# bio-phys/BioEn

Measured on NVIDIA B200. Metric: grad_evals_per_s, higher is better.
Workload: dtype f64

## Files before the change

bioen_b200/csrc/bioen_b200.cu:

```cuda
#include "../../include/bioen_b200.h"

#include <chrono>
#include <cmath>
#include <limits>
#include <memory>
#include <mutex>

#include "batched.cuh"
#include "context.cuh"
#include "gsl_min.cuh"
#include "lbfgs.cuh"

using namespace bioen;

namespace {
thread_local std::string g_last_error;
thread_local int g_error_pending = 0;
int g_fast_flag = 0;

void set_error(const char* where, const std::exception& e) {
    g_last_error = std::string(where) + ": " + e.what();
    g_error_pending = 1;
    fprintf(stderr, "%s\n", g_last_error.c_str());
}
// ... 262 lines not shown
            case BIOEN_B200_OPT_LAZY_GRADIENT: ctx->C.lazy_gradient = value != 0; break;
            case BIOEN_B200_OPT_P2P:
                if (ctx->comm) {
                    if (ctx->comm->is_local() && !value)
                        throw std::invalid_argument("bioen_b200: an in-process group has no NCCL path");
                    ctx->comm->use_p2p = value != 0;
                }
                break;
            case BIOEN_B200_OPT_FUSED_EXCHANGE: ctx->C.fuse_allowed = value != 0; break;
            case BIOEN_B200_OPT_PERSISTENT: ctx->C.persistent_mode = value; break;
            case BIOEN_B200_OPT_LBFGS_GRAM: ctx->C.lbfgs_gram_opt = value != 0; break;
            case BIOEN_B200_OPT_SLICE: ctx->C.slice_mode = value; break;
            case BIOEN_B200_OPT_LBFGS_SMALL: ctx->C.lbfgs_small_opt = value != 0; break;
            case BIOEN_B200_OPT_LBFGS_SPECULATIVE: ctx->C.lbfgs_speculative = value != 0; break;
            case BIOEN_B200_OPT_FETCH_ZEROCOPY: ctx->C.fetch_zero_copy = value != 0; break;
            case BIOEN_B200_OPT_STRUCTURE_MAJOR_ONLY:
                CUDA_CHECK(cudaSetDevice(ctx->C.device));
                if (value) ctx->C.enter_yt_only();
                else if (ctx->C.yt_only)
                    throw std::invalid_argument("bioen_b200: the row-major matrix is gone; create a new context");
                break;
            case BIOEN_B200_OPT_FP32_STORAGE:
                CUDA_CHECK(cudaSetDevice(ctx->C.device));
                ctx->pending_gen = -1;
                if (value) ctx->C.convert_to_fp32();
                else if (ctx->C.storage_fp32)
                    throw std::invalid_argument("bioen_b200: the fp64 matrix was released; upload yTilde again");
                break;
            default: throw std::invalid_argument("bioen_b200: unknown option");
        }
// ... 883 lines not shown
```

bioen_b200/csrc/common.cuh:

```cuda
#pragma once
#include <cuda.h>
#include <cuda_runtime.h>
#include <nvtx3/nvToolsExt.h>
#include <stdint.h>

#include <cstdio>
#include <stdexcept>
#include <string>

namespace bioen {

struct CudaError : std::runtime_error {
    using std::runtime_error::runtime_error;
};

inline void cuda_check(cudaError_t e, const char* what, const char* file, int line) {
    if (e != cudaSuccess) {
        char buf[512];
        snprintf(buf, sizeof buf, "bioen_b200: CUDA error %d (%s) at %s:%d: %s", (int)e, cudaGetErrorString(e),
                 file, line, what);
        throw CudaError(buf);
    }
}
#define CUDA_CHECK(x) ::bioen::cuda_check((x), #x, __FILE__, __LINE__)
// ... 78 lines not shown
}

__device__ __forceinline__ void bulk_load_1d_hint(void* dst, const void* src, uint32_t bytes, uint64_t* bar,
                                                  uint64_t policy) {
    asm volatile(
        "cp.async.bulk.shared::cluster.global.mbarrier::complete_tx::bytes.L2::cache_hint [%0], [%1], %2, [%3], %4;" ::
            "r"(smem_u32(dst)),
        "l"(reinterpret_cast<uint64_t>(src)), "r"(bytes), "r"(smem_u32(bar)), "l"(policy)
        : "memory");
}

__device__ __forceinline__ void prefetch_tensormap(const CUtensorMap* map) {
    asm volatile("prefetch.tensormap [%0];" ::"l"(reinterpret_cast<uint64_t>(map)) : "memory");
}

__device__ __forceinline__ double warp_sum(double v) {
#pragma unroll
    for (int o = 16; o > 0; o >>= 1) v += __shfl_xor_sync(0xffffffffu, v, o);
    return v;
}

__device__ __forceinline__ double warp_max(double v) {
#pragma unroll
    for (int o = 16; o > 0; o >>= 1) v = fmax(v, __shfl_xor_sync(0xffffffffu, v, o));
    return v;
}

template <int K>
__device__ __forceinline__ void block_sum(double (&v)[K], double* red) {
    const int lane = threadIdx.x & 31, wid = threadIdx.x >> 5, nw = (blockDim.x + 31) >> 5;
// ... 114 lines not shown
```

bioen_b200/csrc/context.cuh:

```cuda
#pragma once
#include <cstdlib>
#include <cstring>
#include <string>
#include <thread>
#include <vector>

#include "comm.cuh"
#include "fused_pass.cuh"
#include <atomic>
#include "persistent_eval.cuh"
#include "slice_eval.cuh"
#include "stream_pass.cuh"
#include "vector_kernels.cuh"

namespace bioen {

template <class T>
struct DevBuf {
    T* p = nullptr;
    size_t n = 0;
    DevBuf() = default;
    DevBuf(const DevBuf&) = delete;
    DevBuf& operator=(const DevBuf&) = delete;
    ~DevBuf() { release(); }
// ... 88 lines not shown

    DevBuf<double> Yt, fpart, flse;
    DevBuf<double> lbfgs_store;
    DevBuf<double> lbfgs_gram, lbfgs_gram_partials;
    bool lbfgs_gram_opt = false;
    bool lbfgs_small_opt = true;
    bool lbfgs_speculative = true;
    long long ldt = 0, f_nslab = 0, f_chunk = 0;
    int f_C = 0, f_stages = 0, f_grid = 0, f_KI = 0, f_smem = 0, f_T = 1, f_rows = 0, f_rows_per_cta = 1;
    bool f_team = false;
    bool fused_ready = false, yt_valid = false;
    bool allow_fused = true;
    double theta = 0.0;
    bool have_logw = false, have_forces = false;
    long long passes_launched = 0, kernels_launched = 0;

    Context(int m, int n, int dev, cudaStream_t user_stream = nullptr) : M(m), N(n), N_total(n), device(dev) {
        if (m <= 0 || n <= 0) throw std::invalid_argument("bioen_b200: matrix dimensions must be positive");
        CUDA_CHECK(cudaSetDevice(device));
        cudaDeviceProp prop;
        CUDA_CHECK(cudaGetDeviceProperties(&prop, device));
        if (prop.major < 10)
            throw CudaError("bioen_b200: this library is built for sm_100a (Blackwell B200) only");
        num_sms = prop.multiProcessorCount;
        if (user_stream) {
            stream = user_stream;
            own_stream = false;
        } else {
            CUDA_CHECK(cudaStreamCreateWithFlags(&stream, cudaStreamNonBlocking));
        }
// ... 47 lines not shown
                                        cudaFuncAttributeMaxDynamicSharedMemorySize, kPassSmemBytes));
        CUDA_CHECK(cudaFuncSetAttribute(stream_pass_kernel<kRowPass, false, float>,
                                        cudaFuncAttributeMaxDynamicSharedMemorySize, kPassSmemBytesF32));
        CUDA_CHECK(cudaFuncSetAttribute(stream_pass_kernel<kRowPass, true, float>,
                                        cudaFuncAttributeMaxDynamicSharedMemorySize, kPassSmemBytesF32));
        CUDA_CHECK(cudaFuncSetAttribute(stream_pass_kernel<kColPass, false, float>,
                                        cudaFuncAttributeMaxDynamicSharedMemorySize, kPassSmemBytesF32));
        CUDA_CHECK(cudaFuncSetAttribute(stream_pass_kernel<kColPass, true, float>,
                                        cudaFuncAttributeMaxDynamicSharedMemorySize, kPassSmemBytesF32));
        CUDA_CHECK(cudaFuncSetAttribute(stream_colgrad_kernel<double>, cudaFuncAttributeMaxDynamicSharedMemorySize,
                                        kPassSmemBytes));
        CUDA_CHECK(cudaFuncSetAttribute(stream_colgrad_kernel<float>, cudaFuncAttributeMaxDynamicSharedMemorySize,
                                        kPassSmemBytesF32));
        colgrad_part.alloc((size_t)grid * 3 + 8);
        if (const char* e = getenv("BIOEN_B200_COLGRAD")) colgrad_opt = e[0] != '0';
        CUDA_CHECK(cudaFuncSetAttribute(persistent_eval_kernel<double>, cudaFuncAttributeMaxDynamicSharedMemorySize,
                                        kPassSmemBytes));
        CUDA_CHECK(cudaFuncSetAttribute(persistent_eval_kernel<float>, cudaFuncAttributeMaxDynamicSharedMemorySize,
                                        kPassSmemBytesF32));
        pe_part.alloc((size_t)grid * kPSlots + 16);
        pe_bar.alloc(32);
        {
            int coop = 0, per_sm = 0;
            CUDA_CHECK(cudaDeviceGetAttribute(&coop, cudaDevAttrCooperativeLaunch, device));
            CUDA_CHECK(cudaOccupancyMaxActiveBlocksPerMultiprocessor(&per_sm, persistent_eval_kernel<float>,
                                                                     kPEvalThreads, kPassSmemBytesF32));
            coop_ok = coop && (long long)per_sm * num_sms >= grid;
            if (const char* e = getenv("BIOEN_B200_PERSISTENT")) persistent_mode = atoi(e);
            if (const char* e = getenv("BIOEN_B200_LBFGS_GRAM")) lbfgs_gram_opt = e[0] == '1';
            if (const char* e = getenv("BIOEN_B200_FETCH")) fetch_zero_copy = strcmp(e, "memcpy") != 0;
// ... 43 lines not shown
        lbfgs_gram_opt = getenv("BIOEN_B200_LBFGS_GRAM") != nullptr && getenv("BIOEN_B200_LBFGS_GRAM")[0] == '1';
        lbfgs_small_opt = !(getenv("BIOEN_B200_LBFGS_SMALL") && getenv("BIOEN_B200_LBFGS_SMALL")[0] == '0');
        persistent_mode = -1;
        if (const char* e = getenv("BIOEN_B200_PERSISTENT")) persistent_mode = atoi(e);
        slice_mode = -1;
        if (const char* e = getenv("BIOEN_B200_SLICE")) slice_mode = atoi(e);
        comm = nullptr;
        nranks = 1;
        N_total = N;
        Y = nullptr;
        storage_fp32 = false;
        Y32.release();
        yt_only = false;
        passes_launched = kernels_launched = 0;
        pass_timing = false;
    }
    void set_comm(Comm* c) {
        comm = c;
        nranks = c ? c->nranks : 1;
        if (nranks > 64) throw std::invalid_argument("bioen_b200: at most 64 ranks");
    }

    void upload_matrix(const double* host, size_t ld_host) {
        NvtxRange nvtx("bioen:upload_ytilde");
        ld = round_up(N, 16);
        if (Yown.n != (size_t)M * ld || !Yown.p) {
            Yown.release();
            CUDA_CHECK(cudaMalloc(&Yown.p, (size_t)M * ld * sizeof(double)));
            Yown.n = (size_t)M * ld;
        }
// ... 472 lines not shown
        P2PDev d{};
        d.nranks = 1;
        return d;
    }

    const double* lse_pairs() const { return nranks > 1 ? lse_all.p : sc.p + SC_LSE_MAX; }

    void launch_lse(double* x, const double* xp, const double* d, double stp, const double* w0, bool from_col,
                    const double* stp_dev = nullptr) {
        LseArgs a{};
        a.n = N; a.x = x; a.xp = xp; a.d = d; a.stp = stp; a.stp_dev = stp_dev; a.w0 = w0;
        a.col_partial = from_col ? partialB.p : nullptr;
        a.col_ld = Npad; a.col_L = nRT; a.col_chunk = col_chunk();
        a.write_xnorm = from_col ? 0 : 1;
        a.partials = red_partials.p; a.ticket = ticket.p; a.sc = sc.p;
        k_update_lse<<<vec_blocks_n, kVecThreads, 0, stream>>>(a);
        ++kernels_launched;
    }
    void gather_lse() {
        if (nranks > 1) comm->allgather(sc.p + SC_LSE_MAX, lse_all.p, 2, stream);
    }
    template <int MODE, bool SUB>
    void launch_pass(const double* vN, const double* vMb) {
        PassArgs a{};
        a.nRT = nRT; a.nCB = nCB; a.T = T; a.chunk = chunk;
        a.interleave = ((MODE == kRowPass) ? interleave_row : interleave_col) ? 1 : 0;
        a.evict_first = evict_first;
        a.vN = vN; a.vMb = vMb; a.ab = ab.p;
        a.partial = (MODE == kRowPass) ? partialA.p : partialB.p;
        a.ld = (MODE == kRowPass) ? Mpad : Npad;
        require_row_major("this evaluation path (tile kernels)");
        if (!has_matrix()) throw std::logic_error("bioen_b200: yTilde has not been uploaded");
        const bool timed = pass_timing && pass_ev_used + 2 <= pass_ev.size();
        if (timed) CUDA_CHECK(cudaEventRecord(pass_ev[pass_ev_used++], stream));
        if (storage_fp32)
            stream_pass_kernel<MODE, SUB, float><<<grid, kPassThreads, kPassSmemBytesF32, stream>>>(tmap, a);
        else
            stream_pass_kernel<MODE, SUB, double><<<grid, kPassThreads, kPassSmemBytes, stream>>>(tmap, a);
        if (timed) CUDA_CHECK(cudaEventRecord(pass_ev[pass_ev_used++], stream));
        CUDA_CHECK(cudaGetLastError());
        ++passes_launched;
        ++kernels_launched;
    }
    std::vector<cudaEvent_t> pass_ev;
    size_t pass_ev_used = 0;
    long long pass_ev_passes = 0;
    bool pass_timing = false;
    void begin_pass_timing(int max_passes) {
        while (pass_ev.size() < (size_t)max_passes * 2) {
            cudaEvent_t e;
            CUDA_CHECK(cudaEventCreate(&e));
            pass_ev.push_back(e);
        }
        pass_ev_used = 0;
        pass_ev_passes = 0;
        pass_timing = true;
    }
    float end_pass_timing() {
        pass_timing = false;
        sync();
        double total = 0.0;
        size_t cnt = 0;
        for (size_t i = 0; i + 1 < pass_ev_used; i += 2) {
            float t = 0.f;
            CUDA_CHECK(cudaEventElapsedTime(&t, pass_ev[i], pass_ev[i + 1]));
            total += t;
            ++cnt;
        }
        return cnt ? (float)(total / (double)(cnt + pass_ev_passes)) : 0.f;
    }
    void finalize_rows(bool is_forces, int ntail, bool ab_with_avg) {
        FinalizeArgs a{};
        a.m = M; a.partial = partialA.p; a.ld = Mpad; a.L = nCB; a.chunk = row_chunk();
        a.Y = Yobs.p; a.ab = ab.p; a.avg = avg.p; a.ab_with_avg = ab_with_avg ? 1 : 0;
        a.is_forces = is_forces ? 1 : 0; a.theta = theta;
        a.partials = red_partials.p; a.ticket = ticket.p; a.sc = sc.p;
        a.tail = msum.p + M;
        if (nranks > 1) {
            k_reduce_row_slots<<<vec_blocks_m, kVecThreads, 0, stream>>>(M, partialA.p, Mpad, nCB, row_chunk(), msum.p);
            ++kernels_launched;
            comm->allreduce_sum(msum.p, M + ntail, stream);
            a.msum = msum.p;
        }
        k_finalize_rows<<<(M + kVecThreads - 1) / kVecThreads, kVecThreads, 0, stream>>>(a);
        ++kernels_launched;
    }

    bool slice_ok() const {
        return slice_pl.ok && slice_coop && slice_mode != 0 && persistent_mode != 0 && nranks == 1 && Y != nullptr &&
               !storage_fp32 && (ld % 2) == 0 && ld >= N && (reinterpret_cast<uintptr_t>(Y) & 15) == 0;
    }
    void launch_slice(int method, int mode, double* x, const double* xp, const double* d, double stp,
                      const double* stp_dev, double* grad, const double* ddir) {
        SliceArgs a{};
        a.method = method; a.mode = mode; a.M = M; a.N = N;
        a.nc = slice_pl.nc; a.ncs = slice_pl.ncs; a.ms = slice_pl.ms;
        a.cx_log2 = slice_pl.cx_log2; a.l_log2 = slice_pl.l_log2; a.lt_log2 = slice_pl.lt_log2;
        a.Y = Y; a.ld = ld;
        a.x = x; a.xp = xp; a.d = d; a.stp = stp; a.stp_dev = stp_dev;
// ... 114 lines not shown
        ++eval_gen;
        if (persistent_for(false)) {
            launch_persistent(0, kPEvalObjective, x, xp, d, stp, stp_dev, nullptr, nullptr);
            eval_fused = nranks > 1;
            return;
        }
        launch_lse(x, xp, d, stp, nullptr, false, stp_dev);
        const bool fused = fuse_exchange();
        eval_fused = fused;
        if (!fused) gather_lse();
        {
            LogwWeightsArgs a{};
            a.n = N; a.g = x; a.G = Gv.p; a.w = w.p; a.lse_pairs = lse_pairs(); a.nranks = nranks;
            a.msum_tail = msum.p + M; a.partials = red_partials.p; a.ticket = ticket.p; a.sc = sc.p;
            a.local_only = fused ? 1 : 0;
            k_logw_weights<<<vec_blocks_n, kVecThreads, 0, stream>>>(a);
            ++kernels_launched;
        }
        launch_pass<kRowPass, false>(w.p, nullptr);
        if (fused) {
            RowsExchangeArgs a{};
            a.m = M; a.partial = partialA.p; a.ld = Mpad; a.L = nCB; a.chunk = row_chunk(); a.msum = msum.p;
            a.p2p = p2p_dev(); a.Y = Yobs.p; a.ab = ab.p; a.avg = avg.p; a.theta = theta; a.sc = sc.p;
            k_logw_rows_exchange_finalize<<<1, kRowsXThreads, 0, stream>>>(a);
            ++kernels_launched;
        } else {
            finalize_rows(false, 3, true);
        }
    }
    bool colgrad_eligible() const {
        return colgrad_opt && (nranks == 1 || fuse_exchange()) && interleave_col && !persistent_for(false);
// ... 1 lines not shown
    bool eval_fused = false;
    void logw_eval_g(const double* x, double* grad, const double* ddir) {
        NvtxRange nvtx("bioen:logw_eval_g");
        if (persistent_for(false) && (nranks == 1 || eval_fused)) {
            launch_persistent(0, kPEvalGradient, const_cast<double*>(x), nullptr, nullptr, 0.0, nullptr, grad, ddir);
            eval_fused = false;
            return;
        }
        auto aligned16 = [](const void* q) { return (reinterpret_cast<uintptr_t>(q) & 15) == 0; };
        const bool sharded_fused = nranks > 1 && eval_fused;
        if (colgrad_opt && (nranks == 1 || sharded_fused) && interleave_col && aligned16(x) && aligned16(grad) &&
            aligned16(Gv.p) && aligned16(w.p)) {
            PassArgs pa{};
            pa.nRT = nRT; pa.nCB = nCB; pa.T = T; pa.chunk = chunk; pa.interleave = 1; pa.evict_first = evict_first;
            pa.ab = ab.p; pa.partial = partialB.p; pa.ld = Npad;
            ColGradArgs ga{};
            ga.n = N; ga.g = x; ga.G = Gv.p; ga.w = w.p; ga.d = ddir; ga.grad = grad; ga.theta = theta; ga.sc = sc.p;
            ga.i_gbar = SC_GBAR; ga.i_Gbar = SC_CAPGBAR; ga.cta_part = colgrad_part.p;
            ga.i_wscale = sharded_fused ? SC_WSCALE : -1;
            ga.wio = w.p;
            const bool timed = pass_timing && pass_ev_used + 2 <= pass_ev.size();
            if (timed) CUDA_CHECK(cudaEventRecord(pass_ev[pass_ev_used++], stream));
            if (storage_fp32)
                stream_colgrad_kernel<float><<<grid, kPassThreads, kPassSmemBytesF32, stream>>>(tmap, pa, ga);
            else
                stream_colgrad_kernel<double><<<grid, kPassThreads, kPassSmemBytes, stream>>>(tmap, pa, ga);
            if (timed) CUDA_CHECK(cudaEventRecord(pass_ev[pass_ev_used++], stream));
            CUDA_CHECK(cudaGetLastError());
            if (sharded_fused) k_colgrad_finish_sharded<<<1, 256, 0, stream>>>(grid, colgrad_part.p, sc.p, p2p_dev());
            else k_colgrad_finish<<<1, 256, 0, stream>>>(grid, colgrad_part.p, sc.p, SC_DG, SC_GNORM2, SC_GINF);
            ++passes_launched;
            kernels_launched += 2;
            eval_fused = false;
            return;
        }
        launch_pass<kColPass, true>(nullptr, nullptr);
        {
            LogwGradArgs a{};
            a.n = N; a.col_partial = partialB.p; a.ld = Npad; a.L = nRT; a.chunk = col_chunk();
            a.g = x; a.G = Gv.p; a.w = w.p; a.d = ddir; a.grad = grad; a.theta = theta;
            a.partials = red_partials.p; a.ticket = ticket.p; a.sc = sc.p;
            a.wio = w.p;
            if (eval_fused) a.p2p = p2p_dev(); else a.p2p.nranks = 1;
            k_logw_grad<<<vec_blocks_n, kVecThreads, 0, stream>>>(a);
            ++kernels_launched;
// ... 212 lines not shown
```

bioen_b200/csrc/lbfgs.cuh:

```cuda
#pragma once
#include <chrono>
#include <cmath>
#include <cstdio>
#include <map>

#include "context.cuh"

namespace bioen {

enum {
    LBFGS_SUCCESS = 0,
    LBFGS_STOP = 1,
    LBFGS_ALREADY_MINIMIZED = 2,
    LBFGSERR_UNKNOWNERROR = -1024,
    LBFGSERR_LOGICERROR,
    LBFGSERR_OUTOFMEMORY,
    LBFGSERR_CANCELED,
    LBFGSERR_INVALID_N,
    LBFGSERR_INVALID_N_SSE,
    LBFGSERR_INVALID_X_SSE,
    LBFGSERR_INVALID_EPSILON,
    LBFGSERR_INVALID_TESTPERIOD,
    LBFGSERR_INVALID_DELTA,
    LBFGSERR_INVALID_LINESEARCH,
// ... 429 lines not shown
    LineSearchState* spec_ls = nullptr;
    bool take_spec_slope() {
        if (!spec_slope) return false;
        spec_slope = false;
        const double dg0 = C.h_sc[SC_DGINIT];
        spec_ls->set_slope(dg0);
        spec_bad = 0 < dg0;
        return spec_bad;
    }

    void enqueue_update(int end_old, int bound, int m) {
        NvtxRange nvtx("bioen:lbfgs_update(pair+two_loop)");
        const bool fused = reduce && C.fuse_exchange();
        PairArgs a{n, x, g, xp, gp, S[end_old], Yv[end_old], end_old, C.red_partials.p, C.ticket.p, C.sc.p, {}};
        if (fused) a.p2p = C.p2p_dev(); else a.p2p.nranks = 1;
        k_lbfgs_pair<<<vec_blocks, kVecThreads, 0, C.stream>>>(a);
        ++C.kernels_launched;
        if (reduce && !fused) {
            C.comm->allreduce_sum(C.sc.p + SC_YS, 2, C.stream);
            C.d2d(C.sc.p + SC_YS0 + end_old, C.sc.p + SC_YS, 1);
        }
        two_loop(bound, (end_old + 1) % m, m);
    }
    void enqueue_update_gram(int end_old, int bound) {
        NvtxRange nvtx("bioen:lbfgs_update(gram)");
        GramPairArgs a{};
        a.n = n; a.x = x; a.g = g; a.xp = xp; a.gp = gp;
        for (int t = 0; t < kGramM; ++t) { a.S[t] = S[t]; a.Y[t] = Yv[t]; }
        a.end = end_old; a.bound = bound; a.gram = C.lbfgs_gram.p; a.partials = C.lbfgs_gram_partials.p;
        a.ticket = C.ticket.p; a.sc = C.sc.p;
        if (reduce && C.fuse_exchange()) a.p2p = C.p2p_dev(); else a.p2p.nranks = 1;
// ... 41 lines not shown
                }
                it = g_update.emplace(key, std::make_pair(ex, nk)).first;
            }
            CUDA_CHECK(cudaGraphLaunch(it->second.first, C.stream));
            C.kernels_launched += it->second.second;
            return;
        }
        enqueue_update(end_old, bound, m);
    }

    void two_loop(int bound, int end, int m) {
        const bool fused = reduce && C.fuse_exchange();
        auto launch = [&](TwoLoopArgs& a) {
            a.n = n; a.d = d; a.g = g; a.partials = C.red_partials.p; a.ticket = C.ticket.p; a.sc = C.sc.p;
            if (fused && a.v) a.p2p = C.p2p_dev(); else a.p2p.nranks = 1;
            k_lbfgs_twoloop<<<vec_blocks, kVecThreads, 0, C.stream>>>(a);
            ++C.kernels_launched;
            if (reduce && !fused && a.v) C.comm->allreduce_sum(C.sc.p + a.out, 1, C.stream);
        };
        std::vector<int> js(bound);
        int j = end;
        for (int i = 0; i < bound; ++i) { j = (j + m - 1) % m; js[i] = j; }
        {
            TwoLoopArgs a{};
            a.init = 1; a.u = nullptr; a.c_num = a.c_den = 0; a.c2_num = -1; a.s_num = -1;
            a.v = S[js[0]]; a.out = SC_ALPHA0 + js[0];
            launch(a);
        }
        for (int i = 0; i < bound; ++i) {
            TwoLoopArgs a{};
            a.u = Yv[js[i]]; a.c_num = SC_ALPHA0 + js[i]; a.c_den = SC_YS0 + js[i]; a.csign = -1.0; a.c2_num = -1;
// ... 53 lines not shown
```

bioen_b200/csrc/stream_pass.cuh:

```cuda
#pragma once
#include "common.cuh"

namespace bioen {

enum PassMode { kRowPass = 0, kColPass = 1 };

constexpr int kTileR = 32;
constexpr int kTileC = 128;
#ifndef BIOEN_PASS_STAGES
#define BIOEN_PASS_STAGES 4
#endif
#ifndef BIOEN_PASS_CTAS_PER_SM
#define BIOEN_PASS_CTAS_PER_SM 1
#endif
constexpr int kStages = BIOEN_PASS_STAGES;
constexpr int kPassCtasPerSM = BIOEN_PASS_CTAS_PER_SM;
constexpr int kConsumerWarps = 8;
constexpr int kAuxBytes = 2048;
constexpr int kTileBytes = kTileR * kTileC * (int)sizeof(double);
constexpr int kStageBytes = kTileBytes + kAuxBytes;
constexpr int kPassThreads = (kConsumerWarps + 1) * 32;

template <typename T>
struct PassGeom {
// ... 5 lines not shown
constexpr int kPassSmemBytes = PassGeom<double>::kSmem;
constexpr int kPassSmemBytesF32 = PassGeom<float>::kSmem;

struct PassArgs {
    int nRT;
    int nCB;
    long long T;
    long long chunk;
    int interleave;
    int evict_first;
    const double* vN;
    const double* vMb;
    const double* ab;
    double* partial;
    long long ld;
};

__host__ __device__ inline long long pass_first_cta(long long run, long long L, long long chunk) {
    return chunk < 0 ? 0 : (run * L) / chunk;
}
__host__ __device__ inline int pass_num_slots(long long run, long long L, long long chunk) {
    if (chunk < 0) return (int)(-chunk);
    return (int)(((run + 1) * L - 1) / chunk - (run * L) / chunk) + 1;
}

struct TileWalk {
    long long run, left, L;
    int k, G, mode;
    __host__ __device__ __forceinline__ void init(int pass_mode, const PassArgs& a, int b, int grid) {
        L = (pass_mode == kRowPass) ? a.nCB : a.nRT;
// ... 75 lines not shown
        if (MODE == kRowPass) bytes += kTileC * 8 + (SUB ? kTileR * 8 : 0);
        else bytes += kTileR * 16;
        mbar_expect_tx(&full[stage], bytes);
        tma_load_2d(st, tmap, cb * kTileC, rt * kTileR, &full[stage], policy);
        if (MODE == kRowPass) {
            bulk_load_1d(st + kTileBytes, a.vN + (size_t)cb * kTileC, kTileC * 8, &full[stage]);
            if (SUB)
                bulk_load_1d(st + kTileBytes + kTileC * 8, a.vMb + (size_t)rt * kTileR, kTileR * 8, &full[stage]);
        } else {
            bulk_load_1d(st + kTileBytes, a.ab + (size_t)rt * kTileR * 2, kTileR * 16, &full[stage]);
        }
        if (++stage == kStages) { stage = 0; phase ^= 1; }
    }
    rp.stage = stage;
    rp.phase = phase;
}

template <typename T>
struct RowFrag;
template <>
struct RowFrag<double> {
    double2 v0, v1;
    __device__ __forceinline__ void load_v(const double2* vv, int lane) { v0 = vv[lane]; v1 = vv[32 + lane]; }
    __device__ __forceinline__ double dot(const unsigned char* rowp, int lane, bool sub, double b, double s) const {
        const double2* yr = reinterpret_cast<const double2*>(rowp);
        double2 y0 = yr[lane], y1 = yr[32 + lane];
        if (sub) { y0.x -= b; y0.y -= b; y1.x -= b; y1.y -= b; }
        s = fma(y0.x, v0.x, s);
        s = fma(y0.y, v0.y, s);
        s = fma(y1.x, v1.x, s);
// ... 121 lines not shown
    double* wio;
};

template <typename T>
__global__ void __launch_bounds__(kPassThreads, kPassCtasPerSM)
    stream_colgrad_kernel(const __grid_constant__ CUtensorMap tmap, const PassArgs a, const ColGradArgs ga) {
    using Geo = PassGeom<T>;
    constexpr int kNS = Geo::kNStages, kStageB = Geo::kStage, kTileB = Geo::kTile;
    constexpr int kRowBytes = kTileC * (int)sizeof(T);
    extern __shared__ __align__(1024) unsigned char smem_raw[];
    unsigned char* smem = smem_raw + ((128u - (smem_u32(smem_raw) & 127u)) & 127u);
    __shared__ double s_red[3][kConsumerWarps];
    const int warp = threadIdx.x >> 5, lane = threadIdx.x & 31;
    TileWalk tw;
    tw.init(kColPass, a, (int)blockIdx.x, (int)gridDim.x);
    pass_ring_init<T>(smem);
    __syncthreads();
    if (warp == kConsumerWarps) {
        if (lane == 0 && tw.left > 0) {
            prefetch_tensormap(&tmap);
            RingPos rp{0, 1};
            pass_produce<kColPass, true, T>(smem, &tmap, a, tw, rp);
        }
        return;
    }
    uint64_t* full = reinterpret_cast<uint64_t*>(smem + kNS * kStageB);
    uint64_t* empty = full + kNS;
    constexpr int CPW = kTileC / kConsumerWarps;
    const int cp = lane & 7, rg = lane >> 3;
    const double gbar = ga.sc[ga.i_gbar], Gbar = ga.sc[ga.i_Gbar];
    const double wscale = ga.i_wscale >= 0 ? ga.sc[ga.i_wscale] : 1.0;
// ... 62 lines not shown
            acc0 = acc1 = 0.0;
        }
    }
    dg = warp_sum(dg);
    gn = warp_sum(gn);
    gi = warp_max(gi);
    if (lane == 0) { s_red[0][warp] = dg; s_red[1][warp] = gn; s_red[2][warp] = gi; }
    asm volatile("bar.sync 1, %0;" ::"n"(kConsumerWarps * 32) : "memory");
    if (threadIdx.x == 0) {
        double t0 = 0.0, t1 = 0.0, t2 = 0.0;
        for (int w = 0; w < kConsumerWarps; ++w) { t0 += s_red[0][w]; t1 += s_red[1][w]; t2 = fmax(t2, s_red[2][w]); }
        ga.cta_part[3 * blockIdx.x + 0] = t0;
        ga.cta_part[3 * blockIdx.x + 1] = t1;
        ga.cta_part[3 * blockIdx.x + 2] = t2;
    }
}

__global__ void __launch_bounds__(256) k_colgrad_finish(int ncta, const double* cta_part, double* sc, int i_dg,
                                                        int i_gn, int i_gi) {
    __shared__ double red[3][8];
    double t0 = 0.0, t1 = 0.0, t2 = 0.0;
    for (int b = threadIdx.x; b < ncta; b += 256) {
        t0 += cta_part[3 * b];
        t1 += cta_part[3 * b + 1];
        t2 = fmax(t2, cta_part[3 * b + 2]);
    }
    t0 = warp_sum(t0); t1 = warp_sum(t1); t2 = warp_max(t2);
    if ((threadIdx.x & 31) == 0) { red[0][threadIdx.x >> 5] = t0; red[1][threadIdx.x >> 5] = t1; red[2][threadIdx.x >> 5] = t2; }
    __syncthreads();
    if (threadIdx.x == 0) {
        for (int w = 1; w < 8; ++w) { t0 += red[0][w]; t1 += red[1][w]; t2 = fmax(t2, red[2][w]); }
        sc[i_dg] = t0;
        sc[i_gn] = t1;
        sc[i_gi] = t2;
    }
}

template <int MODE, bool SUB, typename T = double>
__global__ void __launch_bounds__(kPassThreads, kPassCtasPerSM)
    stream_pass_kernel(const __grid_constant__ CUtensorMap tmap, const PassArgs a) {
    extern __shared__ __align__(1024) unsigned char smem_raw[];
    unsigned char* smem = smem_raw + ((128u - (smem_u32(smem_raw) & 127u)) & 127u);
    const int warp = threadIdx.x >> 5, lane = threadIdx.x & 31;
    TileWalk tw;
    tw.init(MODE, a, (int)blockIdx.x, (int)gridDim.x);
    pass_ring_init<T>(smem);
    __syncthreads();
    if (warp == kConsumerWarps) {
        if (lane == 0 && tw.left > 0) {
            prefetch_tensormap(&tmap);
            RingPos rp{0, 1};
            pass_produce<MODE, SUB, T>(smem, &tmap, a, tw, rp);
        }
        return;
    }
    if (tw.left == 0) return;
    RingPos rp{0, 0};
    pass_consume<MODE, SUB, T>(smem, a, tw, rp);
}

}
```

bioen_b200/csrc/vector_kernels.cuh:

```cuda
#pragma once
#include <float.h>

#include "comm.cuh"
#include "common.cuh"
#include "stream_pass.cuh"

namespace bioen {

enum ScalarSlot {
    SC_LSE_MAX = 0,
    SC_LSE_SUM = 1,
    SC_KL = 2,
    SC_GMAX = 3,
    SC_S = 4,
    SC_LOGS0 = 5,
    SC_GBAR = 6,
    SC_CAPGBAR = 7,
    SC_F = 8,
    SC_CHI2 = 9,
    SC_PRIOR = 10,
    SC_DG = 11,
    SC_GNORM2 = 12,
    SC_XNORM2 = 13,
    SC_WSCALE = 14,
// ... 63 lines not shown
    double stp;
    const double* stp_dev;
    const double* w0;
    const double* col_partial;
    long long col_ld;
    long long col_L, col_chunk;
    int write_xnorm;
    double* partials;
    unsigned int* ticket;
    double* sc;
};

__global__ void __launch_bounds__(kVecThreads) k_update_lse(const LseArgs a) {
    __shared__ double red[3 * 32];
    __shared__ bool is_last;
    double m = -DBL_MAX, s = 0.0, xn = 0.0;
    const double stp = a.stp_dev ? __ldg(a.stp_dev) : a.stp;
    for (int j = blockIdx.x * blockDim.x + threadIdx.x; j < a.n; j += gridDim.x * blockDim.x) {
        double x;
        if (a.col_partial) {
            const long long cb = j / kTileC;
            const int ns = pass_num_slots(cb, a.col_L, a.col_chunk);
            x = 0.0;
            for (int q = 0; q < ns; ++q) x += a.col_partial[(size_t)q * a.col_ld + j];
            a.x[j] = x;
        } else if (a.xp) {
            x = fma(stp, a.d[j], a.xp[j]);
            a.x[j] = x;
        } else {
            x = a.x[j];
// ... 43 lines not shown
    int n;
    const double* g;
    const double* G;
    double* w;
    const double* lse_pairs;
    int nranks;
    double* msum_tail;
    double* partials;
    unsigned int* ticket;
    double* sc;
    int local_only;
};

__global__ void __launch_bounds__(kVecThreads) k_logw_weights(const LogwWeightsArgs a) {
    __shared__ double red[3 * 32];
    double M, S;
    if (a.local_only) { M = a.sc[SC_LSE_MAX]; S = 1.0; }
    else global_lse(a.lse_pairs, a.nranks, M, S);
    const double inv = 1.0 / S;
    double v[3] = {0.0, 0.0, 0.0};
    for (int j = blockIdx.x * blockDim.x + threadIdx.x; j < a.n; j += gridDim.x * blockDim.x) {
        const double g = a.g[j], G = a.G[j];
        const double w = exp(g - M) * inv;
        a.w[j] = w;
        v[0] = fma(g - G, w, v[0]);
        v[1] = fma(g, w, v[1]);
        v[2] = fma(G, w, v[2]);
    }
    double* tail = a.msum_tail;
    double* sc = a.sc;
// ... 102 lines not shown
    const double* msum;
    const double* tail;
    const double* Y;
    double* ab;
    double* avg;
    int ab_with_avg;
    int is_forces;
    double theta;
    double* partials;
    unsigned int* ticket;
    double* sc;
};

__global__ void __launch_bounds__(kVecThreads) k_finalize_rows(const FinalizeArgs a) {
    __shared__ double red[32];
    double v[1] = {0.0};
    const int i = blockIdx.x * blockDim.x + threadIdx.x;
    if (i < a.m) {
        double s;
        if (a.msum) {
            s = a.msum[i];
        } else {
            const int ns = pass_num_slots(i / kTileR, a.L, a.chunk);
            s = 0.0;
            for (int q = 0; q < ns; ++q) s += a.partial[(size_t)q * a.ld + i];
        }
        const double r = s - a.Y[i];
        a.avg[i] = s;
        reinterpret_cast<double2*>(a.ab)[i] = make_double2(r, a.ab_with_avg ? s : 0.0);
        v[0] = r * r;
// ... 288 lines not shown
    }
    int fail;
    const double* in = p2p_deliver_and_wait(p, xs, K, &fail);
    if (threadIdx.x == 0) {
#pragma unroll
        for (int k = 0; k < K; ++k) {
            double s = 0.0;
            for (int r = 0; r < p.nranks; ++r) s += __ldcg(in + r * p.cap + k);
            v[k] = fail ? p2p_nan() : s;
        }
    }
}

__global__ void __launch_bounds__(kVecThreads) k_lbfgs_pair(const PairArgs a) {
    __shared__ double red[2 * 32];
    double v[2] = {0.0, 0.0};
    for (int j = blockIdx.x * blockDim.x + threadIdx.x; j < a.n; j += gridDim.x * blockDim.x) {
        const double x = a.x[j], g = a.g[j];
        const double s = x - a.xp[j], y = g - a.gp[j];
        a.s[j] = s;
        a.y[j] = y;
        a.xp[j] = x;
        a.gp[j] = g;
        v[0] = fma(y, s, v[0]);
        v[1] = fma(y, y, v[1]);
    }
    if (!grid_sum_last<2>(v, a.partials, a.ticket, red)) return;
    if (a.p2p.nranks > 1) p2p_sum_inline<2>(a.p2p, v);
    if (threadIdx.x == 0) {
        a.sc[SC_YS] = v[0];
// ... 9 lines not shown
    int init;
    const double* u;
    int c_num, c_den; double csign;
    int c2_num, c2_den; double c2sign;
    int s_num, s_den;
    const double* v;
    int out;
    double* partials;
    unsigned int* ticket;
    double* sc;
    P2PDev p2p;
};

__global__ void __launch_bounds__(kVecThreads) k_lbfgs_twoloop(const TwoLoopArgs a) {
    __shared__ double red[32];
    double coef = 0.0, scale = 1.0;
    if (a.u) {
        coef = a.csign * (a.sc[a.c_num] / a.sc[a.c_den]);
        if (a.c2_num >= 0) coef += a.c2sign * (a.sc[a.c2_num] / a.sc[a.c2_den]);
    }
    if (a.s_num >= 0) scale = a.sc[a.s_num] / a.sc[a.s_den];
    double v[1] = {0.0};
    for (int j = blockIdx.x * blockDim.x + threadIdx.x; j < a.n; j += gridDim.x * blockDim.x) {
        double dj = a.init ? -a.g[j] : a.d[j];
        if (a.u) dj = fma(coef, a.u[j], dj);
        if (a.s_num >= 0) dj *= scale;
        a.d[j] = dj;
        if (a.v) v[0] = fma(a.v[j], dj, v[0]);
    }
    if (a.v) {
// ... 482 lines not shown
```

include/bioen_b200.h:

```cpp
#ifndef BIOEN_B200_H
#define BIOEN_B200_H

#include <stddef.h>

#ifdef __cplusplus
extern "C" {
#endif


typedef struct params_t {
    double *forces;
    double *w0;
    double *g;
    double *G;
    double *yTilde;
    double *YTilde;
    double *w;
    double *result;
    double theta;
    double *yTildeT;
    int caching;
    double *tmp_n;
    double *tmp_m;
    int m;
// ... 77 lines not shown
int bioen_b200_adopt_ytilde(bioen_b200_ctx *ctx, double *yTilde_dev, size_t ld);
int bioen_b200_upload_rows(bioen_b200_ctx *ctx, int row0, int nrows, const double *rows_host, size_t ld);
void *bioen_b200_host_alloc(size_t bytes);
void bioen_b200_host_free(void *p);
int bioen_b200_alloc_ytilde(bioen_b200_ctx *ctx);
int bioen_b200_download_ytilde(bioen_b200_ctx *ctx, int row0, int nrows, long long col0, long long ncols,
                               double *out_host);

int bioen_b200_set_logw(bioen_b200_ctx *ctx, const double *G_host, const double *YTilde_host, double theta);
int bioen_b200_set_forces(bioen_b200_ctx *ctx, const double *w0_host, const double *YTilde_host, double theta);
int bioen_b200_set_theta(bioen_b200_ctx *ctx, double theta);
enum { BIOEN_B200_OPT_FUSED_FORCES = 1, BIOEN_B200_OPT_P2P = 2, BIOEN_B200_OPT_LAZY_GRADIENT = 3,
       BIOEN_B200_OPT_FUSED_EXCHANGE = 4, BIOEN_B200_OPT_PERSISTENT = 5, BIOEN_B200_OPT_LBFGS_GRAM = 6,
       BIOEN_B200_OPT_FP32_STORAGE = 7, BIOEN_B200_OPT_SLICE = 8, BIOEN_B200_OPT_LBFGS_SMALL = 9,
       BIOEN_B200_OPT_LBFGS_SPECULATIVE = 10, BIOEN_B200_OPT_STRUCTURE_MAJOR_ONLY = 11,
       BIOEN_B200_OPT_FETCH_ZEROCOPY = 12 };
int bioen_b200_set_option(bioen_b200_ctx *ctx, int option, int value);

int bioen_b200_eval(bioen_b200_ctx *ctx, int method, const double *x_host, double *f, double *grad_host);
int bioen_b200_grad_continue(bioen_b200_ctx *ctx, int method, double *grad_host);
int bioen_b200_weights(bioen_b200_ctx *ctx, int method, const double *x_host, double *w_host, double *sum);
int bioen_b200_average(bioen_b200_ctx *ctx, const double *w_host, double *avg_host);
int bioen_b200_affine_rows(bioen_b200_ctx *ctx, const double *scale_host, const double *offset_host);
int bioen_b200_forces_from_weights(bioen_b200_ctx *ctx, const double *w_host, double *f, double *grad_host);

int bioen_b200_opt_lbfgs(bioen_b200_ctx *ctx, int method, const double *x0_host, double *x_host,
                         lbfgs_config_params config, visual_params visual, double *fmin, int info[4]);
int bioen_b200_opt_gsl(bioen_b200_ctx *ctx, int method, const double *x0_host, double *x_host,
                       gsl_config_params config, visual_params visual, double *fmin, int info[4]);

int bioen_b200_theta_scan(bioen_b200_ctx *ctx, int method, int K, const double *thetas, const double *x0_host,
// ... 45 lines not shown
```

Baseline: 438.7.

## Use programmatic dependent launch to overlap kernel prologues with predecessors

Launches the pass, colgrad, vector and L-BFGS kernels through cudaLaunchKernelEx with programmatic stream serialization, and adds griddepcontrol launch_dependents/wait calls in the kernels. Each kernel can then start its prologue (tile-walk setup, smem ring init) while the previous kernel is still draining, which hides launch gaps between the many small kernels in each evaluation. Because cudaEvent timing would break overlap, per-pass timing switches to globaltimer stamps written with atomics. The path is on by default for single-rank runs and can be turned off with an env var or an option; it risks ordering bugs if any kernel reads predecessor outputs before its wait.

```diff
diff --git a/bioen_b200/csrc/bioen_b200.cu b/bioen_b200/csrc/bioen_b200.cu
--- a/bioen_b200/csrc/bioen_b200.cu
+++ b/bioen_b200/csrc/bioen_b200.cu
@@ -300,6 +300,7 @@
             case BIOEN_B200_OPT_LBFGS_SMALL: ctx->C.lbfgs_small_opt = value != 0; break;
             case BIOEN_B200_OPT_LBFGS_SPECULATIVE: ctx->C.lbfgs_speculative = value != 0; break;
             case BIOEN_B200_OPT_FETCH_ZEROCOPY: ctx->C.fetch_zero_copy = value != 0; break;
+            case BIOEN_B200_OPT_STREAM_OVERLAP: ctx->C.overlap_opt = value != 0; break;
             case BIOEN_B200_OPT_STRUCTURE_MAJOR_ONLY:
                 CUDA_CHECK(cudaSetDevice(ctx->C.device));
                 if (value) ctx->C.enter_yt_only();
diff --git a/bioen_b200/csrc/common.cuh b/bioen_b200/csrc/common.cuh
--- a/bioen_b200/csrc/common.cuh
+++ b/bioen_b200/csrc/common.cuh
@@ -116,6 +116,21 @@
     asm volatile("prefetch.tensormap [%0];" ::"l"(reinterpret_cast<uint64_t>(map)) : "memory");
 }
 
+__device__ __forceinline__ void griddep_wait() { asm volatile("griddepcontrol.wait;" ::: "memory"); }
+__device__ __forceinline__ void griddep_launch_dependents() {
+    asm volatile("griddepcontrol.launch_dependents;" ::: "memory");
+}
+__device__ __forceinline__ void griddep_enter() {
+    griddep_launch_dependents();
+    griddep_wait();
+}
+
+__device__ __forceinline__ unsigned long long globaltimer_ns() {
+    unsigned long long t;
+    asm volatile("mov.u64 %0, %%globaltimer;" : "=l"(t));
+    return t;
+}
+
 __device__ __forceinline__ double warp_sum(double v) {
 #pragma unroll
     for (int o = 16; o > 0; o >>= 1) v += __shfl_xor_sync(0xffffffffu, v, o);
diff --git a/bioen_b200/csrc/context.cuh b/bioen_b200/csrc/context.cuh
--- a/bioen_b200/csrc/context.cuh
+++ b/bioen_b200/csrc/context.cuh
@@ -126,6 +126,30 @@
     double theta = 0.0;
     bool have_logw = false, have_forces = false;
     long long passes_launched = 0, kernels_launched = 0;
+
+    bool overlap_opt = true;
+    bool overlap() const { return overlap_opt && nranks == 1; }
+    void read_overlap_env() {
+        overlap_opt = !(getenv("BIOEN_B200_OVERLAP") && getenv("BIOEN_B200_OVERLAP")[0] == '0');
+    }
+    template <typename... KArgs, typename... Args>
+    void launch(void (*kernel)(KArgs...), int nblocks, int nthreads, size_t smem, Args&&... args) {
+        if (!overlap()) {
+            kernel<<<nblocks, nthreads, smem, stream>>>(std::forward<Args>(args)...);
+            return;
+        }
+        cudaLaunchAttribute attr{};
+        attr.id = cudaLaunchAttributeProgrammaticStreamSerialization;
+        attr.val.programmaticStreamSerializationAllowed = 1;
+        cudaLaunchConfig_t cfg{};
+        cfg.gridDim = dim3(nblocks);
+        cfg.blockDim = dim3(nthreads);
+        cfg.dynamicSmemBytes = smem;
+        cfg.stream = stream;
+        cfg.attrs = &attr;
+        cfg.numAttrs = 1;
+        CUDA_CHECK(cudaLaunchKernelEx(&cfg, kernel, std::forward<Args>(args)...));
+    }
 
     Context(int m, int n, int dev, cudaStream_t user_stream = nullptr) : M(m), N(n), N_total(n), device(dev) {
         if (m <= 0 || n <= 0) throw std::invalid_argument("bioen_b200: matrix dimensions must be positive");
@@ -203,6 +227,7 @@
                                         kPassSmemBytesF32));
         colgrad_part.alloc((size_t)grid * 3 + 8);
         if (const char* e = getenv("BIOEN_B200_COLGRAD")) colgrad_opt = e[0] != '0';
+        read_overlap_env();
         CUDA_CHECK(cudaFuncSetAttribute(persistent_eval_kernel<double>, cudaFuncAttributeMaxDynamicSharedMemorySize,
                                         kPassSmemBytes));
         CUDA_CHECK(cudaFuncSetAttribute(persistent_eval_kernel<float>, cudaFuncAttributeMaxDynamicSharedMemorySize,
@@ -276,6 +301,7 @@
         yt_only = false;
         passes_launched = kernels_launched = 0;
         pass_timing = false;
+        read_overlap_env();
     }
     void set_comm(Comm* c) {
         comm = c;
@@ -778,7 +804,7 @@
         a.col_ld = Npad; a.col_L = nRT; a.col_chunk = col_chunk();
         a.write_xnorm = from_col ? 0 : 1;
         a.partials = red_partials.p; a.ticket = ticket.p; a.sc = sc.p;
-        k_update_lse<<<vec_blocks_n, kVecThreads, 0, stream>>>(a);
+        launch(k_update_lse, vec_blocks_n, kVecThreads, 0, a);
         ++kernels_launched;
     }
     void gather_lse() {
@@ -793,14 +819,15 @@
         a.vN = vN; a.vMb = vMb; a.ab = ab.p;
         a.partial = (MODE == kRowPass) ? partialA.p : partialB.p;
         a.ld = (MODE == kRowPass) ? Mpad : Npad;
+        a.stamp = next_pass_stamp();
         require_row_major("this evaluation path (tile kernels)");
         if (!has_matrix()) throw std::logic_error("bioen_b200: yTilde has not been uploaded");
-        const bool timed = pass_timing && pass_ev_used + 2 <= pass_ev.size();
+        const bool timed = pass_timing && !overlap() && pass_ev_used + 2 <= pass_ev.size();
         if (timed) CUDA_CHECK(cudaEventRecord(pass_ev[pass_ev_used++], stream));
         if (storage_fp32)
-            stream_pass_kernel<MODE, SUB, float><<<grid, kPassThreads, kPassSmemBytesF32, stream>>>(tmap, a);
+            launch(stream_pass_kernel<MODE, SUB, float>, grid, kPassThreads, kPassSmemBytesF32, tmap, a);
         else
-            stream_pass_kernel<MODE, SUB, double><<<grid, kPassThreads, kPassSmemBytes, stream>>>(tmap, a);
+            launch(stream_pass_kernel<MODE, SUB, double>, grid, kPassThreads, kPassSmemBytes, tmap, a);
         if (timed) CUDA_CHECK(cudaEventRecord(pass_ev[pass_ev_used++], stream));
         CUDA_CHECK(cudaGetLastError());
         ++passes_launched;
@@ -809,6 +836,8 @@
     std::vector<cudaEvent_t> pass_ev;
     size_t pass_ev_used = 0;
     long long pass_ev_passes = 0;
+    DevBuf<unsigned long long> pass_stamp;
+    size_t pass_stamp_used = 0;
     bool pass_timing = false;
     void begin_pass_timing(int max_passes) {
         while (pass_ev.size() < (size_t)max_passes * 2) {
@@ -818,7 +847,16 @@
         }
         pass_ev_used = 0;
         pass_ev_passes = 0;
+        pass_stamp_used = 0;
+        if (overlap()) {
+            if (pass_stamp.n < (size_t)max_passes * 2) pass_stamp.alloc((size_t)max_passes * 2);
+            CUDA_CHECK(cudaMemsetAsync(pass_stamp.p, 0, pass_stamp.n * sizeof(unsigned long long), stream));
+        }
         pass_timing = true;
+    }
+    unsigned long long* next_pass_stamp() {
+        if (!pass_timing || !overlap() || 2 * (pass_stamp_used + 1) > pass_stamp.n) return nullptr;
+        return pass_stamp.p + 2 * pass_stamp_used++;
     }
     float end_pass_timing() {
         pass_timing = false;
@@ -831,6 +869,15 @@
             total += t;
             ++cnt;
         }
+        if (pass_stamp_used) {
+            std::vector<unsigned long long> h(2 * pass_stamp_used);
+            CUDA_CHECK(cudaMemcpy(h.data(), pass_stamp.p, h.size() * sizeof(unsigned long long), cudaMemcpyDeviceToHost));
+            for (size_t i = 0; i < pass_stamp_used; ++i) {
+                const unsigned long long t0 = ~h[2 * i], t1 = h[2 * i + 1];
+                if (t1 > t0) total += (double)(t1 - t0) * 1e-6;
+                ++cnt;
+            }
+        }
         return cnt ? (float)(total / (double)(cnt + pass_ev_passes)) : 0.f;
     }
     void finalize_rows(bool is_forces, int ntail, bool ab_with_avg) {
@@ -846,7 +893,7 @@
             comm->allreduce_sum(msum.p, M + ntail, stream);
             a.msum = msum.p;
         }
-        k_finalize_rows<<<(M + kVecThreads - 1) / kVecThreads, kVecThreads, 0, stream>>>(a);
+        launch(k_finalize_rows, (M + kVecThreads - 1) / kVecThreads, kVecThreads, 0, a);
         ++kernels_launched;
     }
 
@@ -991,7 +1038,7 @@
             a.n = N; a.g = x; a.G = Gv.p; a.w = w.p; a.lse_pairs = lse_pairs(); a.nranks = nranks;
             a.msum_tail = msum.p + M; a.partials = red_partials.p; a.ticket = ticket.p; a.sc = sc.p;
             a.local_only = fused ? 1 : 0;
-            k_logw_weights<<<vec_blocks_n, kVecThreads, 0, stream>>>(a);
+            launch(k_logw_weights, vec_blocks_n, kVecThreads, 0, a);
             ++kernels_launched;
         }
         launch_pass<kRowPass, false>(w.p, nullptr);
@@ -1023,21 +1070,22 @@
             PassArgs pa{};
             pa.nRT = nRT; pa.nCB = nCB; pa.T = T; pa.chunk = chunk; pa.interleave = 1; pa.evict_first = evict_first;
             pa.ab = ab.p; pa.partial = partialB.p; pa.ld = Npad;
+            pa.stamp = next_pass_stamp();
             ColGradArgs ga{};
             ga.n = N; ga.g = x; ga.G = Gv.p; ga.w = w.p; ga.d = ddir; ga.grad = grad; ga.theta = theta; ga.sc = sc.p;
             ga.i_gbar = SC_GBAR; ga.i_Gbar = SC_CAPGBAR; ga.cta_part = colgrad_part.p;
             ga.i_wscale = sharded_fused ? SC_WSCALE : -1;
             ga.wio = w.p;
-            const bool timed = pass_timing && pass_ev_used + 2 <= pass_ev.size();
+            const bool timed = pass_timing && !overlap() && pass_ev_used + 2 <= pass_ev.size();
             if (timed) CUDA_CHECK(cudaEventRecord(pass_ev[pass_ev_used++], stream));
             if (storage_fp32)
-                stream_colgrad_kernel<float><<<grid, kPassThreads, kPassSmemBytesF32, stream>>>(tmap, pa, ga);
+                launch(stream_colgrad_kernel<float>, grid, kPassThreads, kPassSmemBytesF32, tmap, pa, ga);
             else
-                stream_colgrad_kernel<double><<<grid, kPassThreads, kPassSmemBytes, stream>>>(tmap, pa, ga);
+                launch(stream_colgrad_kernel<double>, grid, kPassThreads, kPassSmemBytes, tmap, pa, ga);
             if (timed) CUDA_CHECK(cudaEventRecord(pass_ev[pass_ev_used++], stream));
             CUDA_CHECK(cudaGetLastError());
             if (sharded_fused) k_colgrad_finish_sharded<<<1, 256, 0, stream>>>(grid, colgrad_part.p, sc.p, p2p_dev());
-            else k_colgrad_finish<<<1, 256, 0, stream>>>(grid, colgrad_part.p, sc.p, SC_DG, SC_GNORM2, SC_GINF);
+            else launch(k_colgrad_finish, 1, 256, 0, grid, colgrad_part.p, sc.p, SC_DG, SC_GNORM2, SC_GINF);
             ++passes_launched;
             kernels_launched += 2;
             eval_fused = false;
diff --git a/bioen_b200/csrc/lbfgs.cuh b/bioen_b200/csrc/lbfgs.cuh
--- a/bioen_b200/csrc/lbfgs.cuh
+++ b/bioen_b200/csrc/lbfgs.cuh
@@ -467,7 +467,7 @@
         const bool fused = reduce && C.fuse_exchange();
         PairArgs a{n, x, g, xp, gp, S[end_old], Yv[end_old], end_old, C.red_partials.p, C.ticket.p, C.sc.p, {}};
         if (fused) a.p2p = C.p2p_dev(); else a.p2p.nranks = 1;
-        k_lbfgs_pair<<<vec_blocks, kVecThreads, 0, C.stream>>>(a);
+        C.launch(k_lbfgs_pair, vec_blocks, kVecThreads, 0, a);
         ++C.kernels_launched;
         if (reduce && !fused) {
             C.comm->allreduce_sum(C.sc.p + SC_YS, 2, C.stream);
@@ -539,7 +539,7 @@
         auto launch = [&](TwoLoopArgs& a) {
             a.n = n; a.d = d; a.g = g; a.partials = C.red_partials.p; a.ticket = C.ticket.p; a.sc = C.sc.p;
             if (fused && a.v) a.p2p = C.p2p_dev(); else a.p2p.nranks = 1;
-            k_lbfgs_twoloop<<<vec_blocks, kVecThreads, 0, C.stream>>>(a);
+            C.launch(k_lbfgs_twoloop, vec_blocks, kVecThreads, 0, a);
             ++C.kernels_launched;
             if (reduce && !fused && a.v) C.comm->allreduce_sum(C.sc.p + a.out, 1, C.stream);
         };
diff --git a/bioen_b200/csrc/stream_pass.cuh b/bioen_b200/csrc/stream_pass.cuh
--- a/bioen_b200/csrc/stream_pass.cuh
+++ b/bioen_b200/csrc/stream_pass.cuh
@@ -43,6 +43,7 @@
     const double* ab;
     double* partial;
     long long ld;
+    unsigned long long* stamp;
 };
 
 __host__ __device__ inline long long pass_first_cta(long long run, long long L, long long chunk) {
@@ -148,6 +149,13 @@
     }
     rp.stage = stage;
     rp.phase = phase;
+}
+
+__device__ __forceinline__ void pass_stamp_start(unsigned long long* s) {
+    if (s && threadIdx.x == 0) atomicMax(s, ~globaltimer_ns());
+}
+__device__ __forceinline__ void pass_stamp_end(unsigned long long* s) {
+    if (s && (threadIdx.x & 31) == 0) atomicMax(s + 1, globaltimer_ns());
 }
 
 template <typename T>
@@ -299,7 +307,10 @@
     const int warp = threadIdx.x >> 5, lane = threadIdx.x & 31;
     TileWalk tw;
     tw.init(kColPass, a, (int)blockIdx.x, (int)gridDim.x);
+    griddep_launch_dependents();
     pass_ring_init<T>(smem);
+    griddep_wait();
+    pass_stamp_start(a.stamp);
     __syncthreads();
     if (warp == kConsumerWarps) {
         if (lane == 0 && tw.left > 0) {
@@ -392,11 +403,13 @@
         ga.cta_part[3 * blockIdx.x + 1] = t1;
         ga.cta_part[3 * blockIdx.x + 2] = t2;
     }
+    pass_stamp_end(a.stamp);
 }
 
 __global__ void __launch_bounds__(256) k_colgrad_finish(int ncta, const double* cta_part, double* sc, int i_dg,
                                                         int i_gn, int i_gi) {
     __shared__ double red[3][8];
+    griddep_enter();
     double t0 = 0.0, t1 = 0.0, t2 = 0.0;
     for (int b = threadIdx.x; b < ncta; b += 256) {
         t0 += cta_part[3 * b];
@@ -422,7 +435,10 @@
     const int warp = threadIdx.x >> 5, lane = threadIdx.x & 31;
     TileWalk tw;
     tw.init(MODE, a, (int)blockIdx.x, (int)gridDim.x);
+    griddep_launch_dependents();
     pass_ring_init<T>(smem);
+    griddep_wait();
+    pass_stamp_start(a.stamp);
     __syncthreads();
     if (warp == kConsumerWarps) {
         if (lane == 0 && tw.left > 0) {
@@ -435,6 +451,7 @@
     if (tw.left == 0) return;
     RingPos rp{0, 0};
     pass_consume<MODE, SUB, T>(smem, a, tw, rp);
-}
-
-}
+    pass_stamp_end(a.stamp);
+}
+
+}
diff --git a/bioen_b200/csrc/vector_kernels.cuh b/bioen_b200/csrc/vector_kernels.cuh
--- a/bioen_b200/csrc/vector_kernels.cuh
+++ b/bioen_b200/csrc/vector_kernels.cuh
@@ -101,6 +101,7 @@
 __global__ void __launch_bounds__(kVecThreads) k_update_lse(const LseArgs a) {
     __shared__ double red[3 * 32];
     __shared__ bool is_last;
+    griddep_enter();
     double m = -DBL_MAX, s = 0.0, xn = 0.0;
     const double stp = a.stp_dev ? __ldg(a.stp_dev) : a.stp;
     for (int j = blockIdx.x * blockDim.x + threadIdx.x; j < a.n; j += gridDim.x * blockDim.x) {
@@ -174,6 +175,7 @@
 
 __global__ void __launch_bounds__(kVecThreads) k_logw_weights(const LogwWeightsArgs a) {
     __shared__ double red[3 * 32];
+    griddep_enter();
     double M, S;
     if (a.local_only) { M = a.sc[SC_LSE_MAX]; S = 1.0; }
     else global_lse(a.lse_pairs, a.nranks, M, S);
@@ -306,6 +308,7 @@
 
 __global__ void __launch_bounds__(kVecThreads) k_finalize_rows(const FinalizeArgs a) {
     __shared__ double red[32];
+    griddep_enter();
     double v[1] = {0.0};
     const int i = blockIdx.x * blockDim.x + threadIdx.x;
     if (i < a.m) {
@@ -624,6 +627,7 @@
 
 __global__ void __launch_bounds__(kVecThreads) k_lbfgs_pair(const PairArgs a) {
     __shared__ double red[2 * 32];
+    griddep_enter();
     double v[2] = {0.0, 0.0};
     for (int j = blockIdx.x * blockDim.x + threadIdx.x; j < a.n; j += gridDim.x * blockDim.x) {
         const double x = a.x[j], g = a.g[j];
@@ -663,6 +667,7 @@
 
 __global__ void __launch_bounds__(kVecThreads) k_lbfgs_twoloop(const TwoLoopArgs a) {
     __shared__ double red[32];
+    griddep_enter();
     double coef = 0.0, scale = 1.0;
     if (a.u) {
         coef = a.csign * (a.sc[a.c_num] / a.sc[a.c_den]);
diff --git a/include/bioen_b200.h b/include/bioen_b200.h
--- a/include/bioen_b200.h
+++ b/include/bioen_b200.h
@@ -115,7 +115,7 @@
        BIOEN_B200_OPT_FUSED_EXCHANGE = 4, BIOEN_B200_OPT_PERSISTENT = 5, BIOEN_B200_OPT_LBFGS_GRAM = 6,
        BIOEN_B200_OPT_FP32_STORAGE = 7, BIOEN_B200_OPT_SLICE = 8, BIOEN_B200_OPT_LBFGS_SMALL = 9,
        BIOEN_B200_OPT_LBFGS_SPECULATIVE = 10, BIOEN_B200_OPT_STRUCTURE_MAJOR_ONLY = 11,
-       BIOEN_B200_OPT_FETCH_ZEROCOPY = 12 };
+       BIOEN_B200_OPT_FETCH_ZEROCOPY = 12, BIOEN_B200_OPT_STREAM_OVERLAP = 13 };
 int bioen_b200_set_option(bioen_b200_ctx *ctx, int option, int value);
 
 int bioen_b200_eval(bioen_b200_ctx *ctx, int method, const double *x_host, double *f, double *grad_host);
```

Result: no change. 442.9 (median of 6 runs) (+1.0%).
